# NVIDIA/k8s-operator-libs

Hardware: NVIDIA H100
Metric: node state-transitions/sec (higher is better)
Workload: dtype u8/i32

## Files before the change

k8s-operator-libs_b200/csrc/ust_api.cu:

```cuda
#include <cuda_runtime.h>
#include <dlfcn.h>
#include <nccl.h>

#include <cstdarg>
#include <cstdio>
#include <cstdlib>
#include <cstring>
#include <algorithm>
#include <mutex>
#include <string>
#include <vector>

#include "ust_dev.h"

namespace {

thread_local std::string g_create_error;

struct NcclApi {
  void* lib = nullptr;
  ncclResult_t (*GetUniqueId)(ncclUniqueId*) = nullptr;
  ncclResult_t (*CommInitRank)(ncclComm_t*, int, ncclUniqueId, int) = nullptr;
  ncclResult_t (*AllReduce)(const void*, void*, size_t, ncclDataType_t, ncclRedOp_t, ncclComm_t, cudaStream_t) = nullptr;
  ncclResult_t (*AllGather)(const void*, void*, size_t, ncclDataType_t, ncclComm_t, cudaStream_t) = nullptr;
// ... 100 lines not shown
  int num_sms = 0;
  size_t stream_smem = 0;
  size_t l2_bytes = 0;
  int stream_ctas_per_sm = 0;
  unsigned long long verify_ctas = 0;
  bool ws_dirty = false;
  bool pdl = true;
  bool stamps = false;
  int static_pct = 75;
  unsigned call_seq = 0;
  struct Span { const char* p; size_t len; };
  Span prev_in[4] = {}, prev_out[3] = {};
  int64_t prev_n = -1;
  bool chain_entry = false;
  int64_t relaxed_calls = 0;
  bool overlap_calls = true;
  cudaStream_t last_stream = nullptr;
  int64_t resident_n = -1;
  int32_t resident_n_ds = 0;
  bool outputs_resident = false;
  int64_t pods_n = -1;
  int64_t pods_total = 0;
  DevBuf<ust_counters> sim_hist;
  int segments = 6;
  bool no_hint = false;

  UstWorkspace* ws = nullptr;
  uint32_t* lut_dev = nullptr;
  uint8_t* podlut_dev = nullptr;
  uint32_t* lut_host = nullptr;
  uint8_t* podlut_host = nullptr;
  ust_policy lut_policy;
  bool lut_valid = false;
  ust_counters* counters_dev = nullptr;
  ust_counters* counters_host = nullptr;
  long long* xchg_dev = nullptr;
  DevBuf<unsigned long long> ds_count;

  Columns staged;
  Outputs outs;
  DevBuf<uint8_t> s_outcome, s_outcome_prev;
  DevBuf<int32_t> s_dsrev, s_podoff, s_dsdesired;
  DevBuf<uint16_t> s_rev16;
  DevBuf<int8_t> s_ds8;
  DevBuf<uint16_t> s_podflags;
  DevBuf<uint8_t> s_podsum;
  DevBuf<unsigned int> s_candtile[2];
  Outputs outs_prev, outs_sparse;
  DevBuf<unsigned int> sp_blocks;
  DevBuf<long long> sp_idx;
  long long* sp_count_dev = nullptr;
  long long* sp_count_host = nullptr;
  DevBuf<uint64_t> s_uid, s_dsuid;
  DevBuf<int32_t> s_dsorder;
  IndexedColumns changed;
  DevBuf<long long> pl_idx;
  DevBuf<int32_t> pl_off, pl_shift, pl_runs, s_podoff2;
  DevBuf<uint16_t> pl_flags, s_podflags2;
  DevBuf<uint8_t> sp_outcome;
  std::vector<int32_t> pod_len, pod_len_next, pl_shift_host;
  Columns splice_cols;
  Outputs splice_outs;
  DevBuf<long long> removed, runs;
  IndexedColumns inserted;
  std::vector<long long> run_off, run_src;
  std::vector<uint64_t> run_seen;
// ... 22 lines not shown
    cudaError_t e_ = (call);                                                                                \
    if (e_ != cudaSuccess) return (h)->fail(UST_ERR_CUDA, "%s failed: %s", #call, cudaGetErrorString(e_)); \
  } while (0)

static cudaError_t clear_workspace(ust_handle* h, cudaStream_t st) {
  h->verify_ctas = 0;
  return cudaMemsetAsync(h->ws, 0, sizeof(UstWorkspace), st);
}

static bool policy_active(const ust_policy* p) { return p != nullptr && p->auto_upgrade != 0; }

static ust_policy table_key(const ust_policy* p) {
  ust_policy k;
  memset(&k, 0, sizeof(k));
  if (!policy_active(p)) return k;
  k = *p;
  k.max_parallel_upgrades = 0;
  k.max_unavailable_kind = 0;
  k.max_unavailable_value = 0;
  return k;
}

static int ensure_tables(ust_handle* h, const ust_policy* p, cudaStream_t st) {
  const ust_policy key = table_key(p);
  if (h->lut_valid && memcmp(&key, &h->lut_policy, sizeof(key)) == 0) return UST_OK;
  UST_CUDA(h, cudaStreamSynchronize(st));
  if (policy_active(p)) {
    ust_build_lut(&key, h->lut_host);
    ust_build_pod_lut256(&key, h->podlut_host);
  } else {
    ust_build_lut(nullptr, h->lut_host);
    memset(h->podlut_host, 0, UST_PODLUT_ENTRIES);
  }
  UST_CUDA(h, cudaMemcpyAsync(h->lut_dev, h->lut_host, UST_LUT_WORDS * sizeof(uint32_t), cudaMemcpyHostToDevice, st));
  UST_CUDA(h, cudaMemcpyAsync(h->podlut_dev, h->podlut_host, UST_PODLUT_ENTRIES, cudaMemcpyHostToDevice, st));
  h->lut_policy = key;
  h->lut_valid = true;
  return UST_OK;
}

static int max_grid(const ust_handle* h) { return h->num_sms * UST_STREAM_GRID_PER_SM; }
static int pick_tile_nodes(const ust_handle* h, int64_t n) {
  int tn = UST_TILE_NODES;
  while (tn > 128 && n / tn < (int64_t)max_grid(h)) { tn = (tn / 2) & ~127; if (tn < 128) tn = 128; }
  return tn;
}
static int pick_grid(const ust_handle* h, int tiles) {
  const int g = tiles < max_grid(h) ? tiles : max_grid(h);
  return g < 1 ? 1 : g;
}
static int pick_static_rounds(const ust_handle* h, int tiles, int grid) {
  const int rounds = tiles / grid;
  int r = (int)((int64_t)rounds * h->static_pct / 100);
  if (rounds - r < 2) r = rounds - 2;
  if (r < 1 && rounds >= 1) r = 1;
  return r < 0 ? 0 : r;
}

static int check_aligned(ust_handle* h, const void* p, const char* what) {
  if (((uintptr_t)p & 15u) != 0) return h->fail(UST_ERR_INVALID_ARGUMENT, "%s must be 16-byte aligned", what);
  return UST_OK;
}

static int begin_call(ust_handle* h, const ust_policy* policy, int64_t n, const uint8_t* state, const uint32_t* flags,
                      const int32_t* pod_rev, const int32_t* ds_idx, int32_t n_ds, const int32_t* ds_rev,
                      const int32_t* pod_off, const uint16_t* pod_flags, uint8_t* next_state, uint16_t* actions,
                      uint8_t* outcome, ust_counters* out_dev, cudaStream_t st, UstParams* out, int* grid_out) {
  if (h->last_stream && h->last_stream != st) UST_CUDA(h, cudaStreamSynchronize(h->last_stream));
  h->last_stream = st;
  if (h->ws_dirty) {
    UST_CUDA(h, clear_workspace(h, st));
    h->ws_dirty = false;
  }
  int rc = ensure_tables(h, policy, st);
  if (rc) return rc;
  const bool active = policy_active(policy);
  UstParams P;
  memset(&P, 0, sizeof(P));
  P.n = n;
  P.hot = state; P.flags = flags; P.pod_rev = pod_rev; P.ds_idx = ds_idx;
  P.ds_rev = ds_rev; P.n_ds = n_ds;
  P.pod_off = pod_off; P.pod_flags = pod_flags;
  P.next = next_state; P.actions = actions; P.outcome = outcome;
  P.lut = h->lut_dev; P.podlut = h->podlut_dev;
  P.ws = h->ws; P.xchg = h->xchg_dev;
  P.out = out_dev ? out_dev : h->counters_dev;
  P.active = active ? 1 : 0;
  if (active) {
    P.max_parallel = policy->max_parallel_upgrades;
    P.max_unav_value = policy->max_unavailable_value;
    P.max_unav_kind = policy->max_unavailable_kind;
    P.requestor = policy->use_maintenance_operator != 0;
    P.pd_enabled = policy->pod_deletion_enabled != 0;
    P.pd_spec_present = policy->pod_deletion_spec_present != 0;
    P.eval_pods = (policy->evaluate_actuators != 0 && pod_off) ? 1 : 0;
  }
  P.rank = h->rank;
  P.world = h->world;
  if (h->world > 1 && h->comm_mode == 1 && h->mbox_ready) {
    P.fused_exchange = 1;
    for (int r = 0; r < h->world; r++) P.mbox[r] = h->mbox[r];
  }
  P.split = (h->world > 1 && !P.fused_exchange) ? 1 : 0;
  P.spec_cut_tile = (active && policy->max_parallel_upgrades == 0 && policy->max_unavailable_kind == UST_MAXUNAVAIL_NIL) ? 0x7FFFFFFF : 0;
  const int tn = pick_tile_nodes(h, n);
  const int64_t tiles64 = (n + tn - 1) / tn;
  const int tiles = (int)tiles64;
  const int grid = pick_grid(h, tiles);
  if (active && !P.requestor && !h->no_hint) {
    unsigned long long sig = 1469598103934665603ull;
    const long long parts[6] = {n, tn, policy->max_parallel_upgrades, policy->max_unavailable_kind, policy->max_unavailable_value, h->world * 64 + h->rank};
    for (long long v : parts) { sig ^= (unsigned long long)v; sig *= 1099511628211ull; }
    P.spec_sig = sig ? sig : 1;
  }
  P.tile_nodes = tn;
  P.n_tiles = tiles;
  P.tile_begin = 0;
  P.tile_end = tiles;
  P.static_rounds = pick_static_rounds(h, tiles, grid);
  P.publish = 1;
  P.stamps = (h->stamps && grid <= UST_MAX_CTAS) ? 1 : 0;
  P.evict_first_inputs = (size_t)n * 13u <= h->l2_bytes ? 1 : 0;
  for (auto& b : h->s_candtile) {
    if ((size_t)tiles + 1 > b.cap && h->last_stream) cudaStreamSynchronize(h->last_stream);
    cudaError_t ce = b.reserve((size_t)tiles + 1);
    if (ce != cudaSuccess) return h->fail(UST_ERR_CUDA, "cudaMalloc failed: %s", cudaGetErrorString(ce));
  }
  if (P.fused_exchange) P.epoch = ++h->epoch;
// ... 1144 lines not shown
```

k8s-operator-libs_b200/csrc/ust_dev.h:

```cpp
#pragma once
#include <stdint.h>

#include "../../include/ust.h"
#include "ust_lut.h"

#define UST_THREADS 256
#ifndef UST_VERIFY_THREADS
#define UST_VERIFY_THREADS 384
#endif
#define UST_MAX_CTAS 1024
#define UST_MAX_WORLD 8
#define UST_DS_SMEM_MAX 1024

#ifndef UST_TILE_NODES
#define UST_TILE_NODES 3072
#endif
#ifndef UST_STAGES
#define UST_STAGES 4
#endif
#ifndef UST_CONSUMER_WARPS
#define UST_CONSUMER_WARPS 12
#endif
#define UST_STREAM_THREADS (32 * (1 + UST_CONSUMER_WARPS))
#ifndef UST_STREAM_CTAS_PER_SM
// ... 42 lines not shown

#define UST_KEY(pass, gidx_plus1) ((((unsigned long long)(pass)) << 56) | (unsigned long long)(gidx_plus1))

struct UstParams {
  long long n;
  const uint8_t* hot;
  const uint32_t* flags;
  const int32_t* pod_rev;
  const int32_t* ds_idx;
  const int32_t* ds_rev;
  int n_ds;
  const int32_t* pod_off;
  const uint16_t* pod_flags;
  uint8_t* next;
  uint16_t* actions;
  uint8_t* outcome;
  const uint32_t* lut;
  const uint8_t* podlut;
  uint8_t* podsum;
  UstWorkspace* ws;
  unsigned int* cand_tile;
  long long* xchg;
  ust_counters* out;
  long long max_parallel;
  long long max_unav_value;
  int max_unav_kind;
  int active;
  int requestor;
  int pd_enabled;
  int pd_spec_present;
  int eval_pods;
  int spec_cut_tile;
  unsigned long long spec_sig;
  int rank;
  int world;
  int tile_nodes;
  int n_tiles;
  int tile_begin;
  int tile_end;
  int static_rounds;
  int parity;
  int seg;
  int publish;
  int split;
  int relaxed;
  unsigned long long verify_before;
  int evict_first_inputs;
  int stamps;
  int fused_exchange;
  long long epoch;
  UstMailbox* mbox[UST_MAX_WORLD];
};

int ust_launch_stream(const UstParams& p, int grid, void* stream, int pdl);
int ust_launch_verify(const UstParams& p, int grid, void* stream, int pdl);
int ust_stream_config(int device, int* num_sms, size_t* smem_bytes, int* ctas_per_sm);
int ust_launch_pod_summary(long long n, int active, const uint8_t* hot, const int32_t* pod_off, const uint16_t* pod_flags,
                           long long n_pods, const uint8_t* podlut, uint8_t* podsum, int grid, void* stream);
int ust_launch_build_state(long long n, const uint8_t* hot, const int32_t* ds_idx, int n_ds, const int32_t* ds_desired,
                           unsigned long long* ds_count, UstWorkspace* ws, ust_counters* out, int grid, void* stream);
#ifdef __CUDACC__
__host__ __device__
#endif
static inline unsigned ust_uid_hash(unsigned long long x, unsigned long long y) {
  unsigned h = (unsigned)x * 0x9E3779B9u + (unsigned)(x >> 32) * 0x85EBCA6Bu + (unsigned)y * 0xC2B2AE35u + (unsigned)(y >> 32) * 0x27D4EB2Fu;
  return h ^ (h >> 15);
// ... 37 lines not shown
```

k8s-operator-libs_b200/csrc/ust_kernels.cu:

```cuda
#include <climits>

#include "ust_common.cuh"

using namespace ustd;

namespace {

constexpr int kThreads = UST_THREADS;
constexpr int kWarps = kThreads / 32;
constexpr int kVThreads = UST_VERIFY_THREADS;
constexpr int kVWarps = kVThreads / 32;
constexpr int kVStep = kVThreads * 4;
constexpr uint32_t kLutBytes = UST_LUT_WORDS * sizeof(uint32_t);
constexpr int kSimNone = INT32_MIN;
constexpr int kSimLongAgo = -(1 << 30);
constexpr int kDsSmem = 64;

struct __align__(128) Shared {
  uint32_t lut[UST_LUT_ENTRIES];
  uint2 meta[16];
  unsigned long long mbar;
  unsigned long long xflag;
  int dsrev[kDsSmem + 1];
  unsigned int warp_tot[kVWarps];
// ... 161 lines not shown
    const long long i = base + (long long)j * kVStep + 4 * t;
    if (i >= b1) continue;
    const uint32_t fl[4] = {T.f[j].x, T.f[j].y, T.f[j].z, T.f[j].w};
    const uint32_t rv[4] = {T.r[j].x, T.r[j].y, T.r[j].z, T.r[j].w};
    const uint32_t dv[4] = {T.d[j].x, T.d[j].y, T.d[j].z, T.d[j].w};
    uint32_t e[4];
#pragma unroll
    for (int k = 0; k < 4; k++) {
      const uint32_t hb = (T.h[j] >> (8 * k)) & 0xFFu, p = (T.ps[j] >> (8 * k)) & 0xFFu;
      const uint32_t fk = fl[k] & ~((p & 0x10u) << 12);
      e[k] = node_entry(P, S, ds_smem, hb, fk, (int)rv[k], dv[k], grant | ((p & 1u) << 16) | ((p & 0xEu) << 21));
    }
    uint32_t next4, out4;
    uint2 act4;
    pack4(e, next4, act4, out4);
    __stcs(reinterpret_cast<uint32_t*>(P.next + i), next4);
    __stcs(reinterpret_cast<uint2*>(P.actions + i), act4);
    if (P.outcome) __stcs(reinterpret_cast<uint32_t*>(P.outcome + i), out4);
  }
}
__device__ void uniform_span(const UstParams& P, Shared& S, long long b0, long long b1, uint32_t grant) {
  const bool ds_smem = P.n_ds <= kDsSmem;
  constexpr long long kIter = 2LL * kVStep;
  SpanTile A, B;
  span_load(P, A, b0, b1);
  for (long long base = b0; base < b1; base += 2 * kIter) {
    span_load(P, B, base + kIter, b1);
    span_eval(P, S, A, base, b1, grant, ds_smem);
    span_load(P, A, base + 2 * kIter, b1);
    span_eval(P, S, B, base + kIter, b1, grant, ds_smem);
  }
}

__device__ long long count_candidates(const UstParams& P, Shared& S, long long b0, long long b1) {
  const int t = threadIdx.x;
  unsigned c = 0;
  for (long long i = b0 + 16LL * t; i < b1; i += 16LL * kVThreads) {
    const uint4 x = __ldg(reinterpret_cast<const uint4*>(P.hot + i));
    c += __popc(cand_mask4(x.x)) + __popc(cand_mask4(x.y)) + __popc(cand_mask4(x.z)) + __popc(cand_mask4(x.w));
  }
  c = __reduce_add_sync(kFull, c);
  __syncthreads();
  if ((t & 31) == 0) S.warp_tot[t >> 5] = c;
  __syncthreads();
  long long tot = 0;
#pragma unroll
  for (int w = 0; w < kVWarps; w++) tot += S.warp_tot[w];
  __syncthreads();
  return tot;
}

__device__ void redo_steps(const UstParams& P, Shared& S, int tile, int s0, int s1) {
  const long long t0 = (long long)tile * P.tile_nodes;
  long long t1 = t0 + P.tile_nodes;
  if (t1 > P.n) t1 = P.n;
  const long long b0 = t0 + (long long)s0 * kVStep;
  long long b1 = t0 + (long long)s1 * kVStep;
  if (b1 > t1) b1 = t1;
  if (b0 >= b1) return;
  const bool slotted = P.active && !P.requestor;
  const bool aborting = S.abort_key != ~0ull;
  if (slotted && tile == S.cut) {
    long long running = s0 > 0 ? count_candidates(P, S, t0, b0) : 0;
    for (long long base = b0; base < b1; base += kVStep) general_step<true>(P, S, base, b1, 0u, running);
    return;
  }
  const uint32_t grant = (slotted && tile < S.cut) ? UST_W_GRANTED : 0u;
  long long running = 0, full_end = b0;
  if (!aborting) {
    full_end = b0 + ((b1 - b0) / kVStep) * kVStep;
    if (full_end > b0) uniform_span(P, S, b0, full_end, grant);
  }
  for (long long base = full_end; base < b1; base += kVStep) general_step<false>(P, S, base, b1, grant, running);
}

__device__ void redo_range(const UstParams& P, Shared& S, int ta, int tb) {
  const int tn = P.tile_nodes;
  const int steps_per_tile = (tn + kVStep - 1) / kVStep;
  const bool aborting = S.abort_key != ~0ull;
  if (aborting || tn % kVStep != 0) {
    for (int tile = ta; tile < tb; tile++) { redo_steps(P, S, tile, 0, steps_per_tile); __syncthreads(); }
    return;
  }
  const bool slotted = P.active && !P.requestor;
  const int cut = slotted ? S.cut : 0x7FFFFFFF;
  for (int part = 0; part < 2; part++) {
    const int x = part == 0 ? ta : (cut + 1 > ta ? cut + 1 : ta);
    const int y = part == 0 ? (cut < tb ? cut : tb) : tb;
    if (x >= y) continue;
    const uint32_t grant = (slotted && part == 0) ? UST_W_GRANTED : 0u;
    const long long b0 = (long long)x * tn;
    long long b1 = (long long)y * tn;
    if (b1 > P.n) b1 = P.n;
    const long long full_end = b0 + ((b1 - b0) / kVStep) * kVStep;
    if (full_end > b0) uniform_span(P, S, b0, full_end, grant);
    long long running = 0;
    for (long long base = full_end; base < b1; base += kVStep) general_step<false>(P, S, base, b1, grant, running);
  }
  if (cut >= ta && cut < tb) { __syncthreads(); redo_steps(P, S, cut, 0, steps_per_tile); }
}

static_assert(sizeof(Shared) <= UST_VERIFY_SMEM_MAX, "the streaming kernel's residency arithmetic assumes this bound");

__device__ __forceinline__ void verify_cta_done(const UstParams& P) {
  if (UST_STREAM_CTAS_PER_SM < 2) return;
  __syncthreads();
  if (threadIdx.x == 0) {
    __threadfence();
    atomicAdd(&P.ws->verify_done, 1ull);
  }
}

__global__ void __maxnreg__(UST_VERIFY_MAXREG) ust_verify_kernel(const __grid_constant__ UstParams P) {
  __shared__ Shared S;
  const int t = threadIdx.x;
  if (t == 0) {
    mbar_init(&S.mbar, 1);
    mbar_fence_init();
    mbar_arrive_expect_tx(&S.mbar, kLutBytes);
    bulk_g2s(S.lut, P.lut, kLutBytes, &S.mbar);
  }
  if (P.stamps && t == 0 && (blockIdx.x == 0 || blockIdx.x == gridDim.x - 1)) P.ws->dbg2[blockIdx.x == 0 ? 8 : 9] = now_ns();
  griddep_launch_dependents();
  griddep_wait();
  const bool lead = blockIdx.x == 0;
  if (P.stamps && lead && t == 0) P.ws->dbg2[0] = now_ns();
// ... 37 lines not shown
  if (P.stamps && lead && t == 0) P.ws->dbg2[1] = now_ns();
  decide(P, S.D, lead, !comm_ok);
  if (P.stamps && lead && t == 0) P.ws->dbg2[2] = now_ns();
  const int redo = S.D.redo;
  mbar_wait(&S.mbar, 0);
  if (redo == 0) { verify_cta_done(P); return; }
  if (t == 0) {
    S.redo = redo; S.cut = S.D.cut; S.lo = S.D.lo; S.hi = S.D.hi; S.slots = S.D.slots_left;
    S.abort_key = S.D.abort_key; S.node_offset = S.D.node_offset;
  }
  if (P.n_ds <= kDsSmem)
    for (int i = t; i <= P.n_ds; i += kVThreads) S.dsrev[i] = i < P.n_ds ? __ldg(P.ds_rev + i) : 0;
  __syncthreads();
  int first = S.lo, last = S.hi;
  if (redo == 2) { first = 0; last = P.n_tiles - 1; }
  const int m = last - first + 1;
  const int steps_per_tile = (P.tile_nodes + kVStep - 1) / kVStep;
  if (m >= (int)gridDim.x) {
    const int per = (m + (int)gridDim.x - 1) / (int)gridDim.x;
    const int ta = first + (int)blockIdx.x * per, tb = ta + per < last + 1 ? ta + per : last + 1;
    if (ta < tb) redo_range(P, S, ta, tb);
  } else {
    const int items = m * steps_per_tile;
    for (int it = (int)blockIdx.x; it < items; it += (int)gridDim.x) {
      const int tile = first + it / steps_per_tile, st = it % steps_per_tile;
      redo_steps(P, S, tile, st, st + 1);
      __syncthreads();
    }
  }
  if (P.stamps && lead && t == 0) P.ws->dbg2[3] = now_ns();
  verify_cta_done(P);
}

constexpr int kPodBlock = 4096;
constexpr int kPodChunks = 6;

__global__ void __launch_bounds__(kThreads, 6) ust_pod_summary_kernel(long long n, int active, const uint8_t* __restrict__ hot,
                                                                      const int32_t* __restrict__ pod_off,
                                                                      const uint16_t* __restrict__ pod_flags, long long n_pods,
                                                                      const uint8_t* __restrict__ podlut, uint8_t* __restrict__ podsum) {
  __shared__ __align__(16) uint8_t lut[256];
  __shared__ __align__(16) uint8_t res[kPodBlock];
  __shared__ unsigned short list[kPodBlock];
  __shared__ int cnt;
  const int t = threadIdx.x, lane = t & 31;
  if (t < 64) reinterpret_cast<uint32_t*>(lut)[t] = __ldg(reinterpret_cast<const uint32_t*>(podlut) + t);
  const unsigned char* bytes = reinterpret_cast<const unsigned char*>(pod_flags);
  const long long total_bytes = 2 * n_pods;
  auto load_hot = [&](long long base) -> uint4 {
    const long long i0 = base + 16 * t;
    uint32_t w[4] = {0x0E0E0E0Eu, 0x0E0E0E0Eu, 0x0E0E0E0Eu, 0x0E0E0E0Eu};
    if (i0 + 16 <= n) return __ldg(reinterpret_cast<const uint4*>(hot + i0));
    for (int k = 0; k < 16; k++)
      if (i0 + k < n) w[k >> 2] = (w[k >> 2] & ~(0xFFu << (8 * (k & 3)))) | ((uint32_t)hot[i0 + k] << (8 * (k & 3)));
    return make_uint4(w[0], w[1], w[2], w[3]);
  };
  for (long long base = (long long)blockIdx.x * kPodBlock; base < n; base += (long long)gridDim.x * kPodBlock) {
    if (t == 0) cnt = 0;
    __syncthreads();
    const long long i0 = base + 16 * t;
    const uint4 hv = load_hot(base);
    const uint32_t w[4] = {hv.x, hv.y, hv.z, hv.w};
    unsigned needbits = 0;
    uint32_t init[4];
#pragma unroll
    for (int k = 0; k < 16; k++) {
      const unsigned s = (w[k >> 2] >> (8 * (k & 3))) & 15u;
      const bool need = active && s >= UST_STATE_WAIT_FOR_JOBS_REQUIRED && s <= UST_STATE_DRAIN_REQUIRED;
      const uint32_t b = need ? (((s - UST_STATE_WAIT_FOR_JOBS_REQUIRED) << 6) | (s == UST_STATE_WAIT_FOR_JOBS_REQUIRED ? 0x10u : 0u)) : 0u;
      if ((k & 3) == 0) init[k >> 2] = 0;
      init[k >> 2] |= b << (8 * (k & 3));
      needbits |= (need ? 1u : 0u) << k;
    }
    *reinterpret_cast<uint4*>(res + 16 * t) = make_uint4(init[0], init[1], init[2], init[3]);
    const int mine_cnt = __popc(needbits);
    int incl = mine_cnt;
#pragma unroll
    for (int o = 1; o < 32; o <<= 1) {
      const int v = __shfl_up_sync(kFull, incl, o);
      if (lane >= o) incl += v;
    }
    int wbase = 0;
    if (lane == 31) wbase = atomicAdd(&cnt, incl);
    wbase = __shfl_sync(kFull, wbase, 31);
    int slot = wbase + incl - mine_cnt;
    while (needbits) {
      const int k = __ffs(needbits) - 1;
      needbits &= needbits - 1;
      list[slot++] = (unsigned short)(16 * t + k);
    }
    __syncthreads();
    const int total = cnt;
    for (int q = t; q < total; q += kThreads) {
      const int li = list[q];
      const long long i = base + li;
      const int p0 = __ldg(pod_off + i), p1 = __ldg(pod_off + i + 1);
      const int len = p1 - p0;
      unsigned r = 0;
      const unsigned tag = res[li];
      const unsigned s = UST_STATE_WAIT_FOR_JOBS_REQUIRED + (tag >> 6);
      const uint32_t sel = s == UST_STATE_WAIT_FOR_JOBS_REQUIRED ? (uint32_t)UST_POD_MATCH_WAIT_SELECTOR
                         : (s == UST_STATE_POD_DELETION_REQUIRED ? (uint32_t)UST_POD_MATCH_DELETION_FILTER : (uint32_t)UST_POD_MATCH_DRAIN_SELECTOR);
      const unsigned sat = s == UST_STATE_WAIT_FOR_JOBS_REQUIRED ? UST_PODSUM_WAIT_RUNNING
                         : (s == UST_STATE_POD_DELETION_REQUIRED ? (UST_PODSUM_TO_DELETE | UST_PODSUM_CANNOT_DELETE) : UST_PODSUM_DRAIN_ERROR);
      const long long c0 = (2LL * p0) & ~15LL;
      const int nchunks = len > 0 ? (int)((2LL * p1 - c0 + 15) >> 4) : 0;
      const bool safe = c0 + 16LL * nchunks <= total_bytes;
      if (safe) {
        const uint4* src = reinterpret_cast<const uint4*>(bytes + c0);
        int rel = (int)((c0 >> 1) - p0);
        for (int cb = 0; cb < nchunks; cb += kPodChunks) {
          uint4 x[kPodChunks];
#pragma unroll
          for (int u = 0; u < kPodChunks; u++) x[u] = cb + u < nchunks ? __ldcs(src + cb + u) : make_uint4(0u, 0u, 0u, 0u);
#pragma unroll
          for (int u = 0; u < kPodChunks; u++) {
            if (cb + u < nchunks && (r & sat) != sat) {
              const uint32_t wv[4] = {x[u].x, x[u].y, x[u].z, x[u].w};
#pragma unroll
              for (int e = 0; e < 8; e++) {
                const uint32_t f = (e & 1) ? wv[e >> 1] >> 16 : wv[e >> 1];
                if ((f & sel) && (unsigned)(rel + e) < (unsigned)len) r |= lut[f & 255u];
              }
            }
            rel += 8;
          }
        }
      } else {
        for (int p = p0; p < p1; p++) {
          const uint32_t f = __ldg(pod_flags + p);
          if (f & sel) r |= lut[f & 255u];
        }
      }
      unsigned ps;
      if (s == UST_STATE_WAIT_FOR_JOBS_REQUIRED) ps = 0x10u | (r & UST_PODSUM_WAIT_RUNNING);
      else if (s == UST_STATE_POD_DELETION_REQUIRED) ps = r & (UST_PODSUM_TO_DELETE | UST_PODSUM_CANNOT_DELETE);
      else ps = r & UST_PODSUM_DRAIN_ERROR;
      res[li] = (uint8_t)ps;
    }
    __syncthreads();
    if (i0 + 16 <= n) {
      *reinterpret_cast<uint4*>(podsum + i0) = *reinterpret_cast<const uint4*>(res + 16 * t);
    } else {
      for (int k = 0; k < 16; k++)
        if (i0 + k < n) podsum[i0 + k] = res[16 * t + k];
    }
  }
}

constexpr int kUidTabSmem = 2048;

template <bool UID>
__global__ void __launch_bounds__(kThreads) ust_build_state_uid_kernel(long long n, const uint8_t* __restrict__ hot,
                                                                       const ulonglong2* __restrict__ owner,
                                                                       const int32_t* __restrict__ ds_idx_in, int n_ds,
                                                                       const ulonglong2* __restrict__ ds_tab,
                                                                       const int32_t* __restrict__ ds_tab_idx, int tab_slots,
                                                                       int32_t* __restrict__ ds_idx_out,
                                                                       unsigned long long* ds_count, UstWorkspace* ws) {
  __shared__ ulonglong2 tab[kUidTabSmem];
  __shared__ int ord[kUidTabSmem];
  __shared__ unsigned int cnt_ds[kUidTabSmem / 4];
  __shared__ unsigned long long inc[256];
  __shared__ unsigned int cnt[16];
  const int t = threadIdx.x;
  const bool in_smem = UID ? tab_slots <= kUidTabSmem : n_ds <= kUidTabSmem / 4;
  if (in_smem) {
    if (UID)
      for (int i = t; i < tab_slots; i += kThreads) { tab[i] = ds_tab[i]; ord[i] = ds_tab_idx[i]; }
    for (int i = t; i < n_ds; i += kThreads) cnt_ds[i] = 0;
  }
  {
    const unsigned b = t, code = b & 15u;
    unsigned long long v = 0;
    if (code < 14) {
      v = 1ull << (4 * code);
      if (b & (UST_HOT_UNSCHEDULABLE | UST_HOT_NOT_READY)) v |= 1ull << 56;
      if (code == UST_STATE_UPGRADE_REQUIRED && !(b & UST_HOT_SKIP)) v |= 1ull << 60;
// ... 782 lines not shown
```

k8s-operator-libs_b200/csrc/ust_lut.h:

```cpp
#pragma once
#include <stdint.h>

#include "../../include/ust.h"

#ifdef __CUDACC__
#define UST_HD __host__ __device__
#else
#define UST_HD
#endif

#define UST_W_SKIP (1u << 2)
#define UST_W_UNSCHEDULABLE (1u << 3)
#define UST_W_GRANTED (1u << 4)
#define UST_W_SYNCED (1u << 9)
#define UST_W_PD_HAS (1u << 22)
#define UST_W_PD_MISMATCH (1u << 23)
#define UST_W_DRAIN_ERROR (1u << 24)

UST_HD constexpr int ust_shift_of(int s) {
  switch (s) {
    case 0: case 11: return 3;
    case 1: return 2;
    case 3: return 16;
    case 4: return 22;
// ... 153 lines not shown
      break;
    case UST_STATE_VALIDATION_REQUIRED:
      if (w & UST_F_SAFE_LOAD) a |= UST_A_UNBLOCK_SAFE_LOAD;
      if (w & UST_F_VALIDATION_DONE) ust_uncordon_or_done(w, &next, &a);
      break;
    case UST_STATE_UNCORDON_REQUIRED:
      if (!(w & UST_F_REQUESTOR_MODE)) { a |= UST_A_UNCORDON; next = UST_STATE_DONE; }
      else if (p->use_maintenance_operator) { next = UST_STATE_DONE; a |= UST_A_REQUESTOR_ANNO_CHANGE | UST_A_NM_CREATE_OR_DELETE; }
      break;
    default: break;
  }
  return ust_lut_pack(s, next, a, outcome);
}

static inline void ust_build_lut(const ust_policy* p, uint32_t* lut) {
  for (unsigned i = 0; i < UST_LUT_WORDS; i++) lut[i] = 0;
  for (int s = 0; s < 16; s++) {
    const int sh = ust_shift_of(s), base = ust_base_of(s);
    for (uint32_t key = 0; key < (1u << ust_bits_of(s)); key++) {
      const uint32_t w = (uint32_t)(((uint64_t)key << sh) & 0xFFFFFFFFull);
      lut[base + (int)key] = p ? ust_transition((unsigned)s, w, p) : ust_lut_pack((unsigned)s, (unsigned)s, 0, 0xFF);
    }
    lut[UST_LUT_ENTRIES + 2 * s] = ust_meta_x(s);
    lut[UST_LUT_ENTRIES + 2 * s + 1] = ust_meta_y(s);
  }
}
static inline uint32_t ust_lut_lookup(const uint32_t* lut, unsigned s, uint32_t w) {
  const uint32_t x = lut[UST_LUT_ENTRIES + 2 * s], y = lut[UST_LUT_ENTRIES + 2 * s + 1];
  const uint32_t sh = x & 31u;
  const uint32_t fs = (uint32_t)(((uint64_t)w << 32) >> (32 + sh));
  return lut[((fs & (x >> 16)) | y) >> 2];
}

#define UST_PODLUT_ENTRIES 2048u
#define UST_PODSUM_WAIT_RUNNING 0x01u
#define UST_PODSUM_TO_DELETE 0x02u
#define UST_PODSUM_CANNOT_DELETE 0x04u
#define UST_PODSUM_DRAIN_ERROR 0x08u

static inline bool ust_pod_chain_keeps(unsigned pf, bool force, bool delete_emptydir, bool* is_error) {
  const unsigned phase = pf & UST_POD_PHASE_MASK;
  const bool finished = phase == UST_PHASE_SUCCEEDED || phase == UST_PHASE_FAILED;
  *is_error = false;
  if ((pf & UST_POD_HAS_CONTROLLER) && (pf & UST_POD_CONTROLLED_BY_DS) && !finished) {
    if (pf & UST_POD_DS_MISSING) { if (!force) { *is_error = true; return true; } }
    else return true;
  }
  if (pf & UST_POD_MIRROR) return true;
  if ((pf & UST_POD_HAS_EMPTYDIR) && !finished && !delete_emptydir) { *is_error = true; return true; }
  if (!finished && !(pf & UST_POD_HAS_CONTROLLER) && !force) { *is_error = true; return true; }
  return false;
}

static inline void ust_build_pod_lut(const ust_policy* p, uint8_t* podlut) {
  for (unsigned pf = 0; pf < UST_PODLUT_ENTRIES; pf++) {
    unsigned r = 0;
    const unsigned phase = pf & UST_POD_PHASE_MASK;
    if ((pf & UST_POD_MATCH_WAIT_SELECTOR) && (phase == UST_PHASE_RUNNING || phase == UST_PHASE_PENDING)) r |= UST_PODSUM_WAIT_RUNNING;
    bool err;
    if (pf & UST_POD_MATCH_DELETION_FILTER) {
      r |= UST_PODSUM_TO_DELETE;
      if (ust_pod_chain_keeps(pf, p->pod_deletion_force != 0, p->pod_deletion_delete_emptydir != 0, &err)) r |= UST_PODSUM_CANNOT_DELETE;
    }
    if (pf & UST_POD_MATCH_DRAIN_SELECTOR) {
      ust_pod_chain_keeps(pf, p->drain_force != 0, p->drain_delete_emptydir != 0, &err);
      if (err) r |= UST_PODSUM_DRAIN_ERROR;
// ... 12 lines not shown
```

k8s-operator-libs_b200/csrc/ust_common.cuh:

```cuda
#pragma once
#include <cuda_runtime.h>

#include "ust_dev.h"

namespace ustd {

constexpr unsigned kFull = 0xFFFFFFFFu;

__device__ __forceinline__ uint32_t smem_u32(const void* p) { return (uint32_t)__cvta_generic_to_shared(p); }

__device__ __forceinline__ void mbar_init(unsigned long long* bar, unsigned count) {
  asm volatile("mbarrier.init.shared::cta.b64 [%0], %1;" ::"r"(smem_u32(bar)), "r"(count));
}
__device__ __forceinline__ void mbar_fence_init() {
  asm volatile("fence.mbarrier_init.release.cluster;" ::: "memory");
  asm volatile("fence.proxy.async.shared::cta;" ::: "memory");
}
__device__ __forceinline__ void mbar_arrive(unsigned long long* bar) {
  asm volatile("mbarrier.arrive.shared::cta.b64 _, [%0];" ::"r"(smem_u32(bar)) : "memory");
}
__device__ __forceinline__ void mbar_arrive_expect_tx(unsigned long long* bar, uint32_t bytes) {
  asm volatile("mbarrier.arrive.expect_tx.shared::cta.b64 _, [%0], %1;" ::"r"(smem_u32(bar)), "r"(bytes) : "memory");
}
__device__ __forceinline__ void mbar_wait(unsigned long long* bar, uint32_t parity) {
  uint32_t done = 0;
  while (!done) {
    asm volatile(
        "{\n\t.reg .pred p;\n\t"
        "mbarrier.try_wait.parity.shared::cta.b64 p, [%1], %2;\n\t"
        "selp.u32 %0, 1, 0, p;\n\t}"
        : "=r"(done) : "r"(smem_u32(bar)), "r"(parity) : "memory");
  }
}
__device__ __forceinline__ void bulk_g2s(void* dst, const void* src, uint32_t bytes, unsigned long long* bar) {
  asm volatile("cp.async.bulk.shared::cluster.global.mbarrier::complete_tx::bytes [%0], [%1], %2, [%3];"
               ::"r"(smem_u32(dst)), "l"(src), "r"(bytes), "r"(smem_u32(bar)) : "memory");
}
__device__ __forceinline__ void bulk_g2s_stream(void* dst, const void* src, uint32_t bytes, unsigned long long* bar, uint64_t pol) {
  asm volatile("cp.async.bulk.shared::cluster.global.mbarrier::complete_tx::bytes.L2::cache_hint [%0], [%1], %2, [%3], %4;"
               ::"r"(smem_u32(dst)), "l"(src), "r"(bytes), "r"(smem_u32(bar)), "l"(pol) : "memory");
}
__device__ __forceinline__ uint64_t policy_evict_first() {
  uint64_t p;
  asm volatile("createpolicy.fractional.L2::evict_first.b64 %0, 1.0;" : "=l"(p));
  return p;
}
__device__ __forceinline__ uint64_t policy_evict_normal() {
  uint64_t p;
  asm volatile("createpolicy.fractional.L2::evict_normal.b64 %0, 1.0;" : "=l"(p));
  return p;
}
__device__ __forceinline__ void griddep_launch_dependents() { asm volatile("griddepcontrol.launch_dependents;" ::: "memory"); }
__device__ __forceinline__ void griddep_wait() { asm volatile("griddepcontrol.wait;" ::: "memory"); }

__device__ __forceinline__ unsigned long long now_ns() {
// ... 354 lines not shown
```

k8s-operator-libs_b200/csrc/ust_stream.cu:

```cuda
#include "ust_common.cuh"

using namespace ustd;

namespace {

constexpr int kTile = UST_TILE_NODES;
constexpr int kStages = UST_STAGES;
constexpr int kCW = UST_CONSUMER_WARPS;
constexpr int kThreads = UST_STREAM_THREADS;
constexpr int kGroups = kTile / 128;
constexpr int kGPW = (kGroups + kCW - 1) / kCW;
static_assert(kGroups % kCW == 0 || kCW > kGroups, "consumer warps must divide the groups of a tile");
#ifndef UST_HOT_REP
#define UST_HOT_REP 8
#endif
constexpr int kHotRep = UST_HOT_REP;
static_assert(kHotRep == 1 || kHotRep == 8, "hot-byte table: plain or one replica per bank group");
constexpr int kHotShift = kHotRep == 8 ? 7 : 4;
constexpr uint32_t kHotMask = 0x7Fu << kHotShift;
constexpr uint32_t kLutBytes = UST_LUT_WORDS * sizeof(uint32_t);
static_assert(kLutBytes % 16 == 0, "bulk copies move multiples of 16 bytes");

template <bool PODS>
struct Stage {
// ... 136 lines not shown
                            fl[1], (int)r.y, d.y, grant, lo, hi);
  e[2] = eval_node<DS_SMEM>(P, S, ((x >> (16 - kHotShift)) & kHotMask) | rep_off, (x >> 19) & kW, fl[2], (int)r.z, d.z, grant, lo, hi);
  e[3] = eval_node<DS_SMEM>(P, S, ((x >> (24 - kHotShift)) & kHotMask) | rep_off, (x >> 27) & kW, fl[3], (int)r.w, d.w, grant, lo, hi);
  uint32_t next4, out4;
  uint2 act4;
  pack4(e, next4, act4, out4);
  if (FULL || nv == 4) {
    __stcs(reinterpret_cast<uint32_t*>(P.next + base) + q, next4);
    __stcs(reinterpret_cast<uint2*>(P.actions + base) + q, act4);
    if (OUTCOME) __stcs(reinterpret_cast<uint32_t*>(P.outcome + base) + q, out4);
  } else {
    for (int k = 0; k < nv; k++) {
      P.next[base + 4 * q + k] = (uint8_t)(e[k] >> 16);
      P.actions[base + 4 * q + k] = (uint16_t)e[k];
      if (OUTCOME) P.outcome[base + 4 * q + k] = (uint8_t)(e[k] >> 24);
    }
  }
}

template <bool PODS>
__device__ void produce(const UstParams& P, SS<PODS>& S) {
  const int lane = threadIdx.x;
  const int tn = P.tile_nodes, G = (int)gridDim.x, R = P.static_rounds;
  const int t_end = P.tile_end;
  const int dyn_base = P.tile_begin + R * G;
  const uint64_t pol = P.evict_first_inputs ? policy_evict_first() : policy_evict_normal();
  unsigned int* ticket = &P.ws->ticket[P.parity][P.seg];
  int pA = 0x7FFFFFFF, pB = 0x7FFFFFFF;
  if (lane == 0) {
    if (R == 0) { pA = dyn_base + (int)atomicAdd(ticket, 1u); pB = dyn_base + (int)atomicAdd(ticket, 1u); }
    else if (R == 1) pA = dyn_base + (int)atomicAdd(ticket, 1u);
  }
  bool synced = false;
  uint32_t it = 0;
  for (;; it++) {
    int tile = 0;
    if (lane == 0) {
      const int i = (int)it;
      if (i < R) tile = P.tile_begin + (int)blockIdx.x + i * G;
      else tile = ((i - R) & 1) ? pB : pA;
      if (i + 2 >= R) {
        const int c = dyn_base + (int)atomicAdd(ticket, 1u);
        if ((i + 2 - R) & 1) pB = c; else pA = c;
      }
    }
    tile = __shfl_sync(kFull, tile, 0);
    if (tile >= t_end) break;
    if (it == (uint32_t)kStages && !synced) { __syncthreads(); synced = true; }
    const int s = (int)(it % kStages);
    const uint32_t ph = (it / kStages) & 1u;
    mbar_wait(&S.empty[s], ph ^ 1u);
    Stage<PODS>& st = S.st[s];
    const long long base = (long long)tile * tn;
    const long long rem = P.n - base;
    const int valid = rem < tn ? (int)rem : tn;
    const int v16 = valid & ~15;
    if (valid != v16) {
      const int k = v16 + lane;
      if (k < valid) {
        st.hot[k] = P.hot[base + k];
        st.flags[k] = P.flags[base + k];
        st.rev[k] = P.pod_rev[base + k];
        st.ds[k] = P.ds_idx[base + k];
        if (PODS) st.ps[k] = P.podsum[base + k];
      }
    }
    __syncwarp();
    if (lane == 0) {
      S.tile_of[s] = tile;
      mbar_arrive_expect_tx(&S.full[s], (uint32_t)v16 * (PODS ? 14u : 13u));
      if (v16) {
        bulk_g2s_stream(st.flags, P.flags + base, (uint32_t)v16 * 4u, &S.full[s], pol);
        bulk_g2s_stream(st.rev, P.pod_rev + base, (uint32_t)v16 * 4u, &S.full[s], pol);
        bulk_g2s_stream(st.ds, P.ds_idx + base, (uint32_t)v16 * 4u, &S.full[s], pol);
        bulk_g2s_stream(st.hot, P.hot + base, (uint32_t)v16, &S.full[s], pol);
        if (PODS) bulk_g2s_stream(st.ps, P.podsum + base, (uint32_t)v16, &S.full[s], pol);
      }
    }
  }
  if (!synced) __syncthreads();
  const int s = (int)(it % kStages);
  const uint32_t ph = (it / kStages) & 1u;
  mbar_wait(&S.empty[s], ph ^ 1u);
  if (lane == 0) {
    S.tile_of[s] = -1;
    mbar_arrive(&S.full[s]);
  }
}

template <bool DS_SMEM, bool OUTCOME, bool PODS>
__device__ void consume(const UstParams& P, SS<PODS>& S, int cw) {
  const int lane = threadIdx.x & 31;
  const int tn = P.tile_nodes, groups = tn >> 7;
  const int spec_cut = S.spec_cut;
  uint32_t B[4] = {0, 0, 0, 0};
  int pending = 0;
  unsigned spec_before = 0;
  for (uint32_t it = 0;; it++) {
    const int s = (int)(it % kStages);
    const uint32_t ph = (it / kStages) & 1u;
    mbar_wait(&S.full[s], ph);
    const int tile = *reinterpret_cast<volatile int*>(&S.tile_of[s]);
    if (tile < 0) break;
    if (P.stamps && it == 0 && cw == 0 && lane == 0) P.ws->dbg[P.parity][blockIdx.x][1] = now_ns();
    const Stage<PODS>& st = S.st[s];
    const long long base = (long long)tile * tn;
    const long long rem = P.n - base;
    const int valid = rem < tn ? (int)rem : tn;
    const uint32_t grant = tile < spec_cut ? UST_W_GRANTED : 0u;
    uint32_t lo = 0, hi = 0;
    unsigned mycand = 0;
    if (valid == kTile) {
// ... 21 lines not shown
      mbar_arrive(&S.empty[s]);
    }
    __syncwarp();
    pending += 4 * kGPW;
    if (pending > 255 - 4 * kGPW) { flush_counts(S, B); pending = 0; }
  }
  flush_counts(S, B);
  spec_before = __reduce_add_sync(kFull, spec_before);
  if (lane == 0 && spec_before) atomicAdd(&S.spec_before, spec_before);
}

template <bool DS_SMEM, bool OUTCOME, bool PODS>
__global__ void __maxnreg__(UST_STREAM_MAXREG) ust_stream_kernel(const __grid_constant__ UstParams P) {
  extern __shared__ __align__(128) unsigned char ust_smem[];
  SS<PODS>& S = *reinterpret_cast<SS<PODS>*>(ust_smem);
  const int t = threadIdx.x, warp = t >> 5;
  UstWorkspace* ws = P.ws;
  griddep_launch_dependents();
  if (P.stamps && t == 0) {
    ws->dbg[P.parity][blockIdx.x][0] = now_ns();
    unsigned sm;
    asm volatile("mov.u32 %0, %%smid;" : "=r"(sm));
    ws->dbg_sm[P.parity][blockIdx.x] = sm;
  }
  if (warp == 0) {
    if (t == 0) {
      for (int s = 0; s < kStages; s++) { mbar_init(&S.full[s], 1); mbar_init(&S.empty[s], kCW); }
      mbar_init(&S.lutbar, 1);
      mbar_fence_init();
      mbar_arrive_expect_tx(&S.lutbar, kLutBytes);
      bulk_g2s(S.lut, P.lut, kLutBytes, &S.lutbar);
    }
    __syncwarp();
    if (!P.relaxed) griddep_wait();
    produce<PODS>(P, S);
  } else {
    const int ct = t - 32, cn = kThreads - 32;
    for (int i = ct; i < 128 * kHotRep; i += cn) S.hotent[i] = hot_entry((unsigned)(kHotRep == 8 ? i >> 3 : i));
    if (ct < 16) S.cnt[ct] = 0;
    if (ct >= 32 && ct < 32 + kStages) S.stage_acc[ct - 32] = 0;
    if (!P.relaxed) griddep_wait();
    if (DS_SMEM)
      for (int i = ct; i <= P.n_ds; i += cn) S.dsrev[i] = i < P.n_ds ? __ldg(P.ds_rev + i) : 0;
    if (ct == 0) {
      if (UST_STREAM_CTAS_PER_SM > 1 && P.relaxed) {
        while ((unsigned long long)ld_acquire_gpu(reinterpret_cast<const long long*>(&ws->verify_done)) < P.verify_before)
          __nanosleep(64);
      }
      S.errinv = 0;
      S.spec_before = 0;
      const bool slotted = P.active && !P.requestor;
      const int hs = P.relaxed ? P.parity : P.parity ^ 1;
      const bool hinted = P.spec_sig != 0 && __ldcg(&ws->hint_sig[hs]) == P.spec_sig;
      const int cut = !slotted ? 0 : (hinted ? __ldcg(&ws->hint_cut[hs]) : P.spec_cut_tile);
      S.spec_cut = cut;
      if (blockIdx.x == 0) ws->spec_used[P.parity] = cut;
    }
    __syncthreads();
    mbar_wait(&S.lutbar, 0);
    consume<DS_SMEM, OUTCOME, PODS>(P, S, warp - 1);
  }
  __syncthreads();
  if (P.stamps && t == 0) ws->dbg[P.parity][blockIdx.x][2] = now_ns();
  griddep_wait();
  unsigned long long* acc = ws->acc[P.parity];
  if (blockIdx.x == 0 && P.seg == 0 && t >= 64 && t < 64 + 18 + 1 + UST_MAX_SEGMENTS) {
    const int o = t - 64, q = P.parity ^ 1;
// ... 103 lines not shown
```

Baseline: 179.5 billion.

## Replace verify-pass LUT recomputation with byte-parallel grant flip patch

Analyzes the transition LUT on the host to check whether the grant bit only affects upgrade-required nodes without skip/unschedulable flags, and by a fixed action XOR and fixed next-state. When that holds, the verify/redo pass skips the full LUT evaluation and patches the already-written next/actions arrays with SWAR byte tests over 16-byte vectors, storing only when a matching node is found. This cuts the verify pass to a mostly read-only streaming scan. The cost is extra reads of next/actions, and correctness now depends on the first-pass outputs having been computed as denied.

```diff
diff --git a/k8s-operator-libs_b200/csrc/ust_api.cu b/k8s-operator-libs_b200/csrc/ust_api.cu
--- a/k8s-operator-libs_b200/csrc/ust_api.cu
+++ b/k8s-operator-libs_b200/csrc/ust_api.cu
@@ -156,6 +156,7 @@
   uint8_t* podlut_host = nullptr;
   ust_policy lut_policy;
   bool lut_valid = false;
+  UstGrantFlip lut_flip = {};
   ust_counters* counters_dev = nullptr;
   ust_counters* counters_host = nullptr;
   long long* xchg_dev = nullptr;
@@ -244,6 +245,7 @@
     ust_build_lut(nullptr, h->lut_host);
     memset(h->podlut_host, 0, UST_PODLUT_ENTRIES);
   }
+  h->lut_flip = ust_grant_flip(h->lut_host);
   UST_CUDA(h, cudaMemcpyAsync(h->lut_dev, h->lut_host, UST_LUT_WORDS * sizeof(uint32_t), cudaMemcpyHostToDevice, st));
   UST_CUDA(h, cudaMemcpyAsync(h->podlut_dev, h->podlut_host, UST_PODLUT_ENTRIES, cudaMemcpyHostToDevice, st));
   h->lut_policy = key;
@@ -306,6 +308,12 @@
     P.pd_enabled = policy->pod_deletion_enabled != 0;
     P.pd_spec_present = policy->pod_deletion_spec_present != 0;
     P.eval_pods = (policy->evaluate_actuators != 0 && pod_off) ? 1 : 0;
+  }
+  if (active && !P.requestor && h->lut_flip.ok) {
+    P.flip = 1;
+    P.flip_actions = h->lut_flip.actions;
+    P.flip_next_granted = h->lut_flip.next_granted;
+    P.flip_next_denied = h->lut_flip.next_denied;
   }
   P.rank = h->rank;
   P.world = h->world;
diff --git a/k8s-operator-libs_b200/csrc/ust_dev.h b/k8s-operator-libs_b200/csrc/ust_dev.h
--- a/k8s-operator-libs_b200/csrc/ust_dev.h
+++ b/k8s-operator-libs_b200/csrc/ust_dev.h
@@ -98,6 +98,10 @@
   int eval_pods;
   int spec_cut_tile;
   unsigned long long spec_sig;
+  int flip;
+  uint32_t flip_actions;
+  uint32_t flip_next_granted;
+  uint32_t flip_next_denied;
   int rank;
   int world;
   int tile_nodes;
diff --git a/k8s-operator-libs_b200/csrc/ust_kernels.cu b/k8s-operator-libs_b200/csrc/ust_kernels.cu
--- a/k8s-operator-libs_b200/csrc/ust_kernels.cu
+++ b/k8s-operator-libs_b200/csrc/ust_kernels.cu
@@ -217,6 +217,43 @@
   }
 }
 
+static_assert((UST_HOT_STATE_MASK | UST_HOT_SKIP | UST_HOT_UNSCHEDULABLE) == 0x6Fu && UST_STATE_UPGRADE_REQUIRED == 1,
+              "flip_span's byte test: (hot & 0x6F) == 1");
+__device__ __noinline__ void flip_span(const UstParams& P, long long b0, long long b1, bool granted) {
+  const uint32_t nx4 = (granted ? P.flip_next_granted : P.flip_next_denied) * 0x01010101u;
+  const uint32_t da2 = P.flip_actions * 0x00010001u;
+  for (long long i = b0 + 16LL * threadIdx.x; i < b1; i += 16LL * kVThreads) {
+    if (i + 16 > b1) {
+      for (long long k = i; k < b1; k++) {
+        if ((P.hot[k] & 0x6Fu) != UST_STATE_UPGRADE_REQUIRED) continue;
+        P.next[k] = (uint8_t)nx4;
+        P.actions[k] ^= (uint16_t)P.flip_actions;
+      }
+      break;
+    }
+    const uint4 h = __ldg(reinterpret_cast<const uint4*>(P.hot + i));
+    const uint4 nv = __ldcg(reinterpret_cast<const uint4*>(P.next + i));
+    const uint4 a0 = __ldcg(reinterpret_cast<const uint4*>(P.actions + i)), a1 = __ldcg(reinterpret_cast<const uint4*>(P.actions + i + 8));
+    const uint32_t hw[4] = {h.x, h.y, h.z, h.w};
+    uint32_t nw[4] = {nv.x, nv.y, nv.z, nv.w}, aw[8] = {a0.x, a0.y, a0.z, a0.w, a1.x, a1.y, a1.z, a1.w};
+    uint32_t any = 0;
+#pragma unroll
+    for (int q = 0; q < 4; q++) {
+      const uint32_t y = (hw[q] & 0x6F6F6F6Fu) ^ 0x01010101u;
+      const uint32_t bm = ((~(((y & 0x7F7F7F7Fu) + 0x7F7F7F7Fu) | y) & 0x80808080u) >> 7) * 0xFFu;
+      any |= bm;
+      nw[q] = (nw[q] & ~bm) | (nx4 & bm);
+      aw[2 * q] ^= da2 & __byte_perm(bm, 0u, 0x1100);
+      aw[2 * q + 1] ^= da2 & __byte_perm(bm, 0u, 0x3322);
+    }
+    if (any) {
+      __stcs(reinterpret_cast<uint4*>(P.next + i), make_uint4(nw[0], nw[1], nw[2], nw[3]));
+      __stcs(reinterpret_cast<uint4*>(P.actions + i), make_uint4(aw[0], aw[1], aw[2], aw[3]));
+      __stcs(reinterpret_cast<uint4*>(P.actions + i + 8), make_uint4(aw[4], aw[5], aw[6], aw[7]));
+    }
+  }
+}
+
 __device__ long long count_candidates(const UstParams& P, Shared& S, long long b0, long long b1) {
   const int t = threadIdx.x;
   unsigned c = 0;
@@ -251,6 +288,10 @@
     return;
   }
   const uint32_t grant = (slotted && tile < S.cut) ? UST_W_GRANTED : 0u;
+  if (P.flip && S.redo == 1) {
+    flip_span(P, b0, b1, grant != 0u);
+    return;
+  }
   long long running = 0, full_end = b0;
   if (!aborting) {
     full_end = b0 + ((b1 - b0) / kVStep) * kVStep;
@@ -277,6 +318,10 @@
     const long long b0 = (long long)x * tn;
     long long b1 = (long long)y * tn;
     if (b1 > P.n) b1 = P.n;
+    if (P.flip) {
+      flip_span(P, b0, b1, grant != 0u);
+      continue;
+    }
     const long long full_end = b0 + ((b1 - b0) / kVStep) * kVStep;
     if (full_end > b0) uniform_span(P, S, b0, full_end, grant);
     long long running = 0;
diff --git a/k8s-operator-libs_b200/csrc/ust_lut.h b/k8s-operator-libs_b200/csrc/ust_lut.h
--- a/k8s-operator-libs_b200/csrc/ust_lut.h
+++ b/k8s-operator-libs_b200/csrc/ust_lut.h
@@ -209,6 +209,39 @@
   return lut[((fs & (x >> 16)) | y) >> 2];
 }
 
+struct UstGrantFlip {
+  int ok;
+  uint32_t actions;
+  uint32_t next_granted;
+  uint32_t next_denied;
+};
+static inline UstGrantFlip ust_grant_flip(const uint32_t* lut) {
+  UstGrantFlip f = {1, 0, 0, 0};
+  bool seen = false;
+  for (int s = 0; s < 16; s++) {
+    const int sh = ust_shift_of(s);
+    for (uint32_t key = 0; key < (1u << ust_bits_of(s)); key++) {
+      const uint32_t w = (uint32_t)(((uint64_t)key << sh) & 0xFFFFFFFFull);
+      if (!(w & UST_W_GRANTED)) continue;
+      const uint32_t g = ust_lut_lookup(lut, (unsigned)s, w), d = ust_lut_lookup(lut, (unsigned)s, w & ~UST_W_GRANTED);
+      if (s != UST_STATE_UPGRADE_REQUIRED || (w & (UST_W_SKIP | UST_W_UNSCHEDULABLE))) {
+        if (g != d) f.ok = 0;
+        continue;
+      }
+      const uint32_t delta = g ^ d, ng = (g >> 16) & 0xFFu, nd = (d >> 16) & 0xFFu;
+      if (delta >> 24) f.ok = 0;
+      if (!seen) {
+        f.actions = delta & 0xFFFFu; f.next_granted = ng; f.next_denied = nd;
+        seen = true;
+      } else if ((delta & 0xFFFFu) != f.actions || ng != f.next_granted || nd != f.next_denied) {
+        f.ok = 0;
+      }
+    }
+  }
+  if (!f.ok) f.actions = f.next_granted = f.next_denied = 0;
+  return f;
+}
+
 #define UST_PODLUT_ENTRIES 2048u
 #define UST_PODSUM_WAIT_RUNNING 0x01u
 #define UST_PODSUM_TO_DELETE 0x02u
```

New measurement: 179.5 billion (median of 6 runs). Within noise of the previous version (-0.0%).

## Overlap stream producer prefetch with pod-summary kernel via deferred podsum loads

Applied to the files above, without the earlier changes.

The streaming kernel's producer warp no longer waits on the programmatic grid dependency before issuing its first stages of bulk copies. It loads the independent arrays first, uses expect_tx without arrive, and adds the podsum bytes and arrival only after griddep_wait. The pod-summary kernel now triggers dependent launch on its last block iteration and uses a smaller configurable block (1024 nodes, 4 per thread). The aim is to hide the launch and dependency gap between the two kernels and raise the summary kernel's parallelism. The split mbarrier transaction accounting is subtle, and a wrong count could hang the pipeline or break correctness.

```diff
diff --git a/k8s-operator-libs_b200/csrc/ust_common.cuh b/k8s-operator-libs_b200/csrc/ust_common.cuh
--- a/k8s-operator-libs_b200/csrc/ust_common.cuh
+++ b/k8s-operator-libs_b200/csrc/ust_common.cuh
@@ -21,6 +21,9 @@
 }
 __device__ __forceinline__ void mbar_arrive_expect_tx(unsigned long long* bar, uint32_t bytes) {
   asm volatile("mbarrier.arrive.expect_tx.shared::cta.b64 _, [%0], %1;" ::"r"(smem_u32(bar)), "r"(bytes) : "memory");
+}
+__device__ __forceinline__ void mbar_expect_tx(unsigned long long* bar, uint32_t bytes) {
+  asm volatile("mbarrier.expect_tx.relaxed.cta.shared::cta.b64 [%0], %1;" ::"r"(smem_u32(bar)), "r"(bytes) : "memory");
 }
 __device__ __forceinline__ void mbar_wait(unsigned long long* bar, uint32_t parity) {
   uint32_t done = 0;
diff --git a/k8s-operator-libs_b200/csrc/ust_kernels.cu b/k8s-operator-libs_b200/csrc/ust_kernels.cu
--- a/k8s-operator-libs_b200/csrc/ust_kernels.cu
+++ b/k8s-operator-libs_b200/csrc/ust_kernels.cu
@@ -380,7 +380,12 @@
   verify_cta_done(P);
 }
 
-constexpr int kPodBlock = 4096;
+#ifndef UST_POD_BLOCK
+#define UST_POD_BLOCK 1024
+#endif
+constexpr int kPodBlock = UST_POD_BLOCK;
+constexpr int kPodPer = kPodBlock / kThreads;
+static_assert(kPodPer == 4 || kPodPer == 8 || kPodPer == 16, "pod block: 4, 8 or 16 nodes per thread");
 constexpr int kPodChunks = 6;
 
 __global__ void __launch_bounds__(kThreads, 6) ust_pod_summary_kernel(long long n, int active, const uint8_t* __restrict__ hot,
@@ -395,24 +400,36 @@
   if (t < 64) reinterpret_cast<uint32_t*>(lut)[t] = __ldg(reinterpret_cast<const uint32_t*>(podlut) + t);
   const unsigned char* bytes = reinterpret_cast<const unsigned char*>(pod_flags);
   const long long total_bytes = 2 * n_pods;
-  auto load_hot = [&](long long base) -> uint4 {
-    const long long i0 = base + 16 * t;
-    uint32_t w[4] = {0x0E0E0E0Eu, 0x0E0E0E0Eu, 0x0E0E0E0Eu, 0x0E0E0E0Eu};
-    if (i0 + 16 <= n) return __ldg(reinterpret_cast<const uint4*>(hot + i0));
-    for (int k = 0; k < 16; k++)
+  auto load_hot = [&](long long base, uint32_t (&w)[kPodPer / 4]) {
+    const long long i0 = base + kPodPer * t;
+    if (i0 + kPodPer <= n) {
+      if (kPodPer == 16) {
+        const uint4 v = __ldg(reinterpret_cast<const uint4*>(hot + i0));
+        w[0] = v.x; w[1 % (kPodPer / 4)] = v.y; w[2 % (kPodPer / 4)] = v.z; w[3 % (kPodPer / 4)] = v.w;
+      } else if (kPodPer == 8) {
+        const uint2 v = __ldg(reinterpret_cast<const uint2*>(hot + i0));
+        w[0] = v.x; w[1 % (kPodPer / 4)] = v.y;
+      } else {
+        w[0] = __ldg(reinterpret_cast<const uint32_t*>(hot + i0));
+      }
+      return;
+    }
+#pragma unroll
+    for (int j = 0; j < kPodPer / 4; j++) w[j] = 0x0E0E0E0Eu;
+    for (int k = 0; k < kPodPer; k++)
       if (i0 + k < n) w[k >> 2] = (w[k >> 2] & ~(0xFFu << (8 * (k & 3)))) | ((uint32_t)hot[i0 + k] << (8 * (k & 3)));
-    return make_uint4(w[0], w[1], w[2], w[3]);
   };
   for (long long base = (long long)blockIdx.x * kPodBlock; base < n; base += (long long)gridDim.x * kPodBlock) {
+    if (base + (long long)gridDim.x * kPodBlock >= n) griddep_launch_dependents();
     if (t == 0) cnt = 0;
     __syncthreads();
-    const long long i0 = base + 16 * t;
-    const uint4 hv = load_hot(base);
-    const uint32_t w[4] = {hv.x, hv.y, hv.z, hv.w};
+    const long long i0 = base + kPodPer * t;
+    uint32_t w[kPodPer / 4];
+    load_hot(base, w);
     unsigned needbits = 0;
-    uint32_t init[4];
-#pragma unroll
-    for (int k = 0; k < 16; k++) {
+    uint32_t init[kPodPer / 4];
+#pragma unroll
+    for (int k = 0; k < kPodPer; k++) {
       const unsigned s = (w[k >> 2] >> (8 * (k & 3))) & 15u;
       const bool need = active && s >= UST_STATE_WAIT_FOR_JOBS_REQUIRED && s <= UST_STATE_DRAIN_REQUIRED;
       const uint32_t b = need ? (((s - UST_STATE_WAIT_FOR_JOBS_REQUIRED) << 6) | (s == UST_STATE_WAIT_FOR_JOBS_REQUIRED ? 0x10u : 0u)) : 0u;
@@ -420,7 +437,8 @@
       init[k >> 2] |= b << (8 * (k & 3));
       needbits |= (need ? 1u : 0u) << k;
     }
-    *reinterpret_cast<uint4*>(res + 16 * t) = make_uint4(init[0], init[1], init[2], init[3]);
+#pragma unroll
+    for (int j = 0; j < kPodPer / 4; j++) reinterpret_cast<uint32_t*>(res + kPodPer * t)[j] = init[j];
     const int mine_cnt = __popc(needbits);
     int incl = mine_cnt;
 #pragma unroll
@@ -435,7 +453,7 @@
     while (needbits) {
       const int k = __ffs(needbits) - 1;
       needbits &= needbits - 1;
-      list[slot++] = (unsigned short)(16 * t + k);
+      list[slot++] = (unsigned short)(kPodPer * t + k);
     }
     __syncthreads();
     const int total = cnt;
@@ -487,11 +505,13 @@
       res[li] = (uint8_t)ps;
     }
     __syncthreads();
-    if (i0 + 16 <= n) {
-      *reinterpret_cast<uint4*>(podsum + i0) = *reinterpret_cast<const uint4*>(res + 16 * t);
+    if (i0 + kPodPer <= n) {
+      if (kPodPer == 16) *reinterpret_cast<uint4*>(podsum + i0) = *reinterpret_cast<const uint4*>(res + 16 * t);
+      else if (kPodPer == 8) *reinterpret_cast<uint2*>(podsum + i0) = *reinterpret_cast<const uint2*>(res + 8 * t);
+      else *reinterpret_cast<uint32_t*>(podsum + i0) = *reinterpret_cast<const uint32_t*>(res + 4 * t);
     } else {
-      for (int k = 0; k < 16; k++)
-        if (i0 + k < n) podsum[i0 + k] = res[16 * t + k];
+      for (int k = 0; k < kPodPer; k++)
+        if (i0 + k < n) podsum[i0 + k] = res[kPodPer * t + k];
     }
   }
 }
diff --git a/k8s-operator-libs_b200/csrc/ust_stream.cu b/k8s-operator-libs_b200/csrc/ust_stream.cu
--- a/k8s-operator-libs_b200/csrc/ust_stream.cu
+++ b/k8s-operator-libs_b200/csrc/ust_stream.cu
@@ -192,6 +192,26 @@
     else if (R == 1) pA = dyn_base + (int)atomicAdd(ticket, 1u);
   }
   bool synced = false;
+  bool waited = !PODS;
+  auto add_podsum = [&](int s) {
+    Stage<PODS>& st = S.st[s];
+    const long long base = (long long)S.tile_of[s] * tn;
+    const long long rem = P.n - base;
+    const int valid = rem < tn ? (int)rem : tn;
+    const int v16 = valid & ~15;
+    if (v16 + lane < valid) st.ps[v16 + lane] = P.podsum[base + v16 + lane];
+    __syncwarp();
+    if (lane == 0) {
+      mbar_arrive_expect_tx(&S.full[s], (uint32_t)v16);
+      if (v16) bulk_g2s_stream(st.ps, P.podsum + base, (uint32_t)v16, &S.full[s], pol);
+    }
+  };
+  auto wait_pods = [&](uint32_t filled) {
+    griddep_wait();
+    __syncwarp();
+    for (uint32_t k = 0; k < filled; k++) add_podsum((int)k);
+    waited = true;
+  };
   uint32_t it = 0;
   for (;; it++) {
     int tile = 0;
@@ -206,6 +226,7 @@
     }
     tile = __shfl_sync(kFull, tile, 0);
     if (tile >= t_end) break;
+    if (PODS && !waited && it == (uint32_t)kStages) wait_pods(it);
     if (it == (uint32_t)kStages && !synced) { __syncthreads(); synced = true; }
     const int s = (int)(it % kStages);
     const uint32_t ph = (it / kStages) & 1u;
@@ -222,22 +243,24 @@
         st.flags[k] = P.flags[base + k];
         st.rev[k] = P.pod_rev[base + k];
         st.ds[k] = P.ds_idx[base + k];
-        if (PODS) st.ps[k] = P.podsum[base + k];
+        if (PODS && waited) st.ps[k] = P.podsum[base + k];
       }
     }
     __syncwarp();
     if (lane == 0) {
       S.tile_of[s] = tile;
-      mbar_arrive_expect_tx(&S.full[s], (uint32_t)v16 * (PODS ? 14u : 13u));
+      if (waited) mbar_arrive_expect_tx(&S.full[s], (uint32_t)v16 * (PODS ? 14u : 13u));
+      else mbar_expect_tx(&S.full[s], (uint32_t)v16 * 13u);
       if (v16) {
         bulk_g2s_stream(st.flags, P.flags + base, (uint32_t)v16 * 4u, &S.full[s], pol);
         bulk_g2s_stream(st.rev, P.pod_rev + base, (uint32_t)v16 * 4u, &S.full[s], pol);
         bulk_g2s_stream(st.ds, P.ds_idx + base, (uint32_t)v16 * 4u, &S.full[s], pol);
         bulk_g2s_stream(st.hot, P.hot + base, (uint32_t)v16, &S.full[s], pol);
-        if (PODS) bulk_g2s_stream(st.ps, P.podsum + base, (uint32_t)v16, &S.full[s], pol);
-      }
-    }
-  }
+        if (PODS && waited) bulk_g2s_stream(st.ps, P.podsum + base, (uint32_t)v16, &S.full[s], pol);
+      }
+    }
+  }
+  if (PODS && !waited) wait_pods(it);
   if (!synced) __syncthreads();
   const int s = (int)(it % kStages);
   const uint32_t ph = (it / kStages) & 1u;
@@ -325,7 +348,7 @@
       bulk_g2s(S.lut, P.lut, kLutBytes, &S.lutbar);
     }
     __syncwarp();
-    if (!P.relaxed) griddep_wait();
+    if (!PODS && !P.relaxed) griddep_wait();
     produce<PODS>(P, S);
   } else {
     const int ct = t - 32, cn = kThreads - 32;
```

Measured after the change: 185.2 billion before, 184.8 billion after, median of 6. Within noise of the previous version (-0.2%).
